# frutiemax92/YAT

Measured on AMD Instinct MI355X. Metric: images/sec (whole node) SANA-1.6B 1024px bf16 training step, higher is better.
Workload: dtype bf16; 1 GPU; train_sana.py: SANA-1.6B (D=2240, 20 blocks) 1024px, bf16, full fine-tune, cached latents/text embeds, aspect buckets [(32, 32), (16, 64), (24, 42), (44, 22)] round-robin, prompts of 20..300 tokens (text rows packed: the masked padding rows to T=512 are not computed), AdamW+clip; global_batch=8, per_gpu_batch=8, seq_len=1024, parallelism=dp1, num_layers=20, params=1604462784

## Files before the change

### include/yat_hip.h

```cpp
#ifndef YAT_HIP_H
#define YAT_HIP_H
#include <stdint.h>
#ifdef __cplusplus
extern "C" {
#endif

typedef void* yat_stream_t;

#define YAT_OK 0
#define YAT_EINVAL (-1)
#define YAT_ENOCOMM (-2)
#define YAT_ECOMM_BASE 1000

int yat_version(void);

typedef struct yat_gemm_epilogue {
    uint32_t struct_size;
    const void* bias;
    void* aux_out;
    int activation;
    const void* gate;
    const void* residual;
    int ld_aux, ld_gate, ld_residual, rows_per_batch;
    const void* glu_u;
// ... 125 lines not shown
int yat_add_pos_embed(int64_t rows, int N, int D, const void* x, const float* pos, void* out, yat_stream_t stream);
int yat_ddpm_add_noise(int B, int64_t per_sample, const void* x, const void* noise, const void* sqrt_alpha_prod,
                       const void* sqrt_one_minus_alpha_prod, void* noisy, yat_stream_t stream);
int yat_mse_bf16_chunk(int B, int64_t used, int64_t stride, const void* pred, const void* target, float gscale, float* loss,
                       void* dpred, float* workspace_256, yat_stream_t stream);

int yat_hadamard_scale(int rows, int cols, const void* a, int lda, const void* b, int ldb, float scale, void* out, int ldo,
                       yat_stream_t stream);
int yat_hadamard_bwd(int rows, int cols, const void* dd, int ldd, const void* a1, int ld1, const void* a2, int ld2, float scale,
                     void* t1, int ldt1, void* t2, int ldt2, yat_stream_t stream);

int yat_dora_delta(int rows, int cols, const void* W, int ldw, const void* lw, int ldl, const void* mag, float scaling,
                   void* delta, int ldd, float* s_buf, float* n_buf, yat_stream_t stream);
int yat_dora_bwd(int rows, int cols, const void* dd, int ldd, const void* W, int ldw, const void* lw, int ldl, float scaling,
                 const float* s_buf, const float* n_buf, void* t1, int ldt, void* dmag, yat_stream_t stream);

int yat_qknorm_concat_fwd(int B, int N, int T, int H, int dh, float eps, const void* qkv_img, int ld_img, const void* qkv_txt,
                          int ld_txt, const void* wq_img, const void* wk_img, const void* wq_txt, const void* wk_txt,
                          void* joint, int ld_joint, float* rstd, yat_stream_t stream);
uint64_t yat_qknorm_concat_bwd_workspace_bytes(int B, int N, int T, int dh);
int yat_qknorm_concat_bwd(int B, int N, int T, int H, int dh, const void* qkv_img, int ld_img, const void* qkv_txt, int ld_txt,
                          const void* wq_img, const void* wk_img, const void* wq_txt, const void* wk_txt, const float* rstd,
                          const void* d_joint, int ld_dj, void* dqkv_img, int ld_dimg, void* dqkv_txt, int ld_dtxt,
                          void* dwq_img, void* dwk_img, void* dwq_txt, void* dwk_txt, int accumulate_dw, void* workspace,
                          yat_stream_t stream);
int yat_joint_rows(int B, int N, int T, int C, void* joint, int ld_joint, void* img, int ld_img, void* txt, int ld_txt,
                   int to_joint, yat_stream_t stream);

uint64_t yat_gradnorm_workspace_bytes(int64_t n, int nseg);
int yat_gradnorm_clip(int64_t n, const void* grad, int nseg, const int64_t* seg_start, float max_norm, float* norm_out,
                      float* clip_coef, void* workspace, yat_stream_t stream);
int yat_gradnorm_pieces_partial(const void* grad, int npiece, const int64_t* piece_start, const int* chunk_base,
                                int max_piece_chunks, const unsigned char* owned, float* partial, yat_stream_t stream);
int yat_gradnorm_pieces_finish(int ntensor, const int* tensor_first_piece, const int* chunk_base, const float* partial,
                               float max_norm, float* norm_out, float* clip_coef, yat_stream_t stream);
int yat_adamw_step(int64_t n, void* param, void* grad, void* exp_avg, void* exp_avg_sq, const float* clip_coef,
                   double lr, double beta1, double beta2, double eps, double weight_decay, int step, int zero_grad,
                   void* ema_shadow, double ema_decay, int background, yat_stream_t stream);

int yat_dcae_conv3x3(int B, int H, int W, int Cin, int Cout, int upsample, int silu, const void* x, const void* w,
                     const void* bias, int shortcut_mode, const void* shortcut, int shortcut_channels, const void* residual,
                     int out_nchw, void* y, yat_stream_t stream);
int yat_dcae_msla_aggregate(int B, int H, int W, int C3, const void* qkv, const void* w_dw, const void* w_pw, void* out,
                            yat_stream_t stream);
int yat_dcae_rmsnorm_bias(int M, int D, float eps, const void* x, const void* w, const void* b, const void* residual,
                          int relu, void* y, yat_stream_t stream);
int yat_dcae_image_to_uint8(int64_t n, const void* x, void* out, yat_stream_t stream);

int yat_dcae_conv3x3_down(int B, int H, int W, int Cin, int Cout, const void* x, const void* w, const void* bias,
                          int shortcut, void* y, yat_stream_t stream);
int yat_dcae_conv3x3_mean(int B, int H, int W, int Cin, int Cout, const void* x, const void* w, const void* bias,
                          int shortcut, void* y, yat_stream_t stream);
int yat_dcae_image_from_uint8(int64_t npix, const void* x, const void* table, void* out, yat_stream_t stream);

uint64_t yat_vae_groupnorm_workspace_bytes(int B, int HW, int C, int G);
int yat_vae_groupnorm(int B, int HW, int C, int G, float eps, const void* x, const void* w, const void* b, int silu, void* y,
                      void* workspace, yat_stream_t stream);
int yat_vae_attn_fwd(int B, int N, int dh, const void* q, const void* k, const void* v, int ld, void* out, int ldo,
                     yat_stream_t stream);

#define YAT_PLAN_MAX_ARGS 30
#define YAT_PLAN_EVENT_RECORD (-1)
#define YAT_PLAN_STREAM_WAIT_EVENT (-2)
typedef union yat_plan_arg { int64_t i; double d; void* p; } yat_plan_arg;
typedef struct yat_plan_entry { int32_t op; int32_t nargs; yat_plan_arg a[YAT_PLAN_MAX_ARGS]; } yat_plan_entry;
int yat_plan_op_id(const char* name);
// ... 24 lines not shown
```

### yat_amd/csrc/optim.hip

```cpp
#include "common.hpp"
#include "../../include/yat_hip.h"
#include <math.h>

namespace {

constexpr int64_t NORM_CHUNK = 1 << 18;

__global__ __launch_bounds__(256) void gradnorm_partial_kernel(const bf16_t* g, const int64_t* seg_start, int maxchunks,
                                                               float* partial) {
    const int seg = blockIdx.y, ck = blockIdx.x;
    const int64_t s0 = seg_start[seg], s1 = seg_start[seg + 1];
    const int64_t c0 = s0 + (int64_t)ck * NORM_CHUNK;
    if (c0 >= s1) return;
    const int64_t c1 = (c0 + NORM_CHUNK < s1) ? c0 + NORM_CHUNK : s1;
    float s = 0.f;
    const int64_t nvec = (c1 - c0) >> 3;
    for (int64_t i = threadIdx.x; i < nvec; i += 256) {
        float v[8];
        unpack8(*reinterpret_cast<const u32x4*>(g + c0 + i * 8), v);
#pragma unroll
        for (int e = 0; e < 8; ++e) s += v[e] * v[e];
    }
    for (int64_t i = c0 + (nvec << 3) + threadIdx.x; i < c1; i += 256) { const float v = bf2f(g[i]); s += v * v; }
    __shared__ float red[4];
    s = wave_sum(s);
    if ((threadIdx.x & 63) == 0) red[threadIdx.x >> 6] = s;
    __syncthreads();
    if (threadIdx.x == 0) partial[(int64_t)seg * maxchunks + ck] = red[0] + red[1] + red[2] + red[3];
}

__global__ __launch_bounds__(256) void gradnorm_final_kernel(int nseg, const int64_t* seg_start, int maxchunks,
                                                             const float* partial, float max_norm, float* norm_out,
                                                             float* clip_coef) {
    float acc = 0.f;
    for (int seg = threadIdx.x; seg < nseg; seg += 256) {
        const int64_t len = seg_start[seg + 1] - seg_start[seg];
        const int nck = (int)((len + NORM_CHUNK - 1) / NORM_CHUNK);
        float s = 0.f;
        for (int c = 0; c < nck; ++c) s += partial[(int64_t)seg * maxchunks + c];
        const float nb = rbf(sqrtf(s));
        acc += nb * nb;
    }
    __shared__ float red[4];
    acc = wave_sum(acc);
    if ((threadIdx.x & 63) == 0) red[threadIdx.x >> 6] = acc;
    __syncthreads();
    if (threadIdx.x == 0) {
        const float total = rbf(sqrtf(red[0] + red[1] + red[2] + red[3]));
        float coef = rbf(max_norm / rbf(total + 1e-6f));
        coef = coef > 1.0f ? 1.0f : coef;
        norm_out[0] = total;
        clip_coef[0] = coef;
    }
}

__global__ __launch_bounds__(256) void gradnorm_pieces_partial_kernel(const bf16_t* g, const int64_t* piece_start,
                                                                      const int* chunk_base, const unsigned char* owned,
                                                                      float* partial) {
    const int pc = blockIdx.y, ck = blockIdx.x;
    const int nck = chunk_base[pc + 1] - chunk_base[pc];
    if (ck >= nck) return;
    float* dst = partial + chunk_base[pc] + ck;
    if (owned && !owned[pc]) {
        if (threadIdx.x == 0) *dst = 0.f;
        return;
    }
    const int64_t s1 = piece_start[pc + 1];
    const int64_t c0 = piece_start[pc] + (int64_t)ck * NORM_CHUNK;
    const int64_t c1 = (c0 + NORM_CHUNK < s1) ? c0 + NORM_CHUNK : s1;
    float s = 0.f;
    const int64_t nvec = (c1 - c0) >> 3;
    for (int64_t i = threadIdx.x; i < nvec; i += 256) {
        float v[8];
        unpack8(*reinterpret_cast<const u32x4*>(g + c0 + i * 8), v);
#pragma unroll
        for (int e = 0; e < 8; ++e) s += v[e] * v[e];
    }
    for (int64_t i = c0 + (nvec << 3) + threadIdx.x; i < c1; i += 256) { const float v = bf2f(g[i]); s += v * v; }
    __shared__ float red[4];
    s = wave_sum(s);
    if ((threadIdx.x & 63) == 0) red[threadIdx.x >> 6] = s;
    __syncthreads();
    if (threadIdx.x == 0) *dst = red[0] + red[1] + red[2] + red[3];
}

__global__ __launch_bounds__(256) void gradnorm_pieces_final_kernel(int ntensor, const int* tensor_first_piece,
                                                                    const int* chunk_base, const float* partial,
                                                                    float max_norm, float* norm_out, float* clip_coef) {
    float acc = 0.f;
    for (int t = threadIdx.x; t < ntensor; t += 256) {
        float s = 0.f;
        for (int pc = tensor_first_piece[t]; pc < tensor_first_piece[t + 1]; ++pc) {
            float sp = 0.f;
            for (int c = chunk_base[pc]; c < chunk_base[pc + 1]; ++c) sp += partial[c];
            s += sp;
        }
        const float nb = rbf(sqrtf(s));
        acc += nb * nb;
    }
    __shared__ float red[4];
    acc = wave_sum(acc);
    if ((threadIdx.x & 63) == 0) red[threadIdx.x >> 6] = acc;
    __syncthreads();
    if (threadIdx.x == 0) {
        const float total = rbf(sqrtf(red[0] + red[1] + red[2] + red[3]));
        float coef = rbf(max_norm / rbf(total + 1e-6f));
        coef = coef > 1.0f ? 1.0f : coef;
        norm_out[0] = total;
        clip_coef[0] = coef;
    }
}

struct AdamP {
    float wd_mul, w1, beta2, om_b2, bc2_sqrt, eps, neg_step_size, ema_omd;
    int use_wd, zero_grad;
};

__device__ __forceinline__ void adamw_elem(float& pr, float g, float& mr_, float& vr_, float coef, bool clip, const AdamP& a) {
    const float gr = clip ? rbf(g * coef) : g;
    if (a.use_wd) pr = rbf(pr * a.wd_mul);
    const float mr = rbf(mr_ + a.w1 * (gr - mr_));
    float vr = rbf(vr_ * a.beta2);
    vr = rbf(vr + a.om_b2 * gr * gr);
    float den = rbf(sqrtf(vr));
    den = rbf(den / a.bc2_sqrt);
    den = rbf(den + a.eps);
    pr = rbf(pr + a.neg_step_size * mr / den);
// ... 84 lines not shown
        if (a.zero_grad) *reinterpret_cast<u32x2*>(g + i * 4) = u32x2{0u, 0u};
    }
}

}

extern "C" {

static int norm_maxchunks(int64_t n) { return (int)((n + NORM_CHUNK - 1) / NORM_CHUNK); }

uint64_t yat_gradnorm_workspace_bytes(int64_t n, int nseg) {
    return (uint64_t)nseg * norm_maxchunks(n) * sizeof(float);
}

int yat_gradnorm_clip(int64_t n, const void* grad, int nseg, const int64_t* seg_start, float max_norm, float* norm_out,
                      float* clip_coef, void* workspace, yat_stream_t stream) {
    if (n <= 0 || nseg <= 0 || nseg > 65535 || !grad || !seg_start || !norm_out || !clip_coef || !workspace)
        return YAT_EINVAL;
    const int mc = norm_maxchunks(n);
    hipLaunchKernelGGL(gradnorm_partial_kernel, dim3(mc, nseg), dim3(256), 0, (hipStream_t)stream, (const bf16_t*)grad,
                       seg_start, mc, (float*)workspace);
    YAT_CHECK_LAUNCH();
    hipLaunchKernelGGL(gradnorm_final_kernel, dim3(1), dim3(256), 0, (hipStream_t)stream, nseg, seg_start, mc,
                       (const float*)workspace, max_norm, norm_out, clip_coef);
    YAT_CHECK_LAUNCH();
    return YAT_OK;
}

int yat_gradnorm_pieces_partial(const void* grad, int npiece, const int64_t* piece_start, const int* chunk_base,
                                int max_piece_chunks, const unsigned char* owned, float* partial, yat_stream_t stream) {
    if (!grad || npiece <= 0 || npiece > 65535 || !piece_start || !chunk_base || max_piece_chunks <= 0 || !partial)
        return YAT_EINVAL;
    hipLaunchKernelGGL(gradnorm_pieces_partial_kernel, dim3(max_piece_chunks, npiece), dim3(256), 0, (hipStream_t)stream,
                       (const bf16_t*)grad, piece_start, chunk_base, owned, partial);
    YAT_CHECK_LAUNCH();
    return YAT_OK;
}

int yat_gradnorm_pieces_finish(int ntensor, const int* tensor_first_piece, const int* chunk_base, const float* partial,
                               float max_norm, float* norm_out, float* clip_coef, yat_stream_t stream) {
    if (ntensor <= 0 || !tensor_first_piece || !chunk_base || !partial || !norm_out || !clip_coef) return YAT_EINVAL;
    hipLaunchKernelGGL(gradnorm_pieces_final_kernel, dim3(1), dim3(256), 0, (hipStream_t)stream, ntensor, tensor_first_piece,
                       chunk_base, partial, max_norm, norm_out, clip_coef);
    YAT_CHECK_LAUNCH();
    return YAT_OK;
}

int yat_adamw_step(int64_t n, void* param, void* grad, void* exp_avg, void* exp_avg_sq, const float* clip_coef, double lr,
                   double beta1, double beta2, double eps, double weight_decay, int step, int zero_grad, void* ema_shadow,
                   double ema_decay, int background, yat_stream_t stream) {
    if (n <= 0 || (n & 7) || step < 1 || !param || !grad || !exp_avg || !exp_avg_sq) return YAT_EINVAL;
    const double dlr = lr, db1 = beta1, db2 = beta2;
    AdamP a;
    a.use_wd = weight_decay != 0.0;
    a.wd_mul = (float)(1.0 - dlr * weight_decay);
    a.w1 = (float)(1.0 - db1);
    a.beta2 = (float)db2;
    a.om_b2 = (float)(1.0 - db2);
    const double bc1 = 1.0 - pow(db1, (double)step), bc2 = 1.0 - pow(db2, (double)step);
    a.bc2_sqrt = (float)sqrt(bc2);
    a.neg_step_size = (float)(-(dlr / bc1));
    a.eps = (float)eps;
    a.ema_omd = (float)(1.0 - ema_decay);
    a.zero_grad = zero_grad;
    if (background) {
        const int64_t nvec4 = n >> 2;
        int64_t nbg = (nvec4 + 255) / 256;
// ... 26 lines not shown
```

### yat_amd/flat.py

```python
from __future__ import annotations

import math
import os
from types import SimpleNamespace

import torch
import torch.nn as nn

from . import ops

BF16 = torch.bfloat16


class _Node(nn.Module):
    """Anonymous container so parameter names can carry the diffusers dotted paths."""


def schedule(chains):
    serial = os.environ.get("YAT_SERIAL", "0") != "0"
    return (not serial), (1 if serial else int(chains))


def isolate_streams():
    import torch.distributed as dist
# ... 39 lines not shown


class FlatParamModule(nn.Module):
    def _alloc_flat(self, specs, device, bucket_first=None):
        self.dev = torch.device(device)
        offs, off = [], 0
        for name, shape in specs:
            if bucket_first is not None and bucket_first(name):
                off = (off + SHARD_ALIGN - 1) // SHARD_ALIGN * SHARD_ALIGN
            offs.append(off)
            off += (math.prod(shape) + 7) // 8 * 8
        if bucket_first is not None:
            off = (off + SHARD_ALIGN - 1) // SHARD_ALIGN * SHARD_ALIGN
        self.numel_flat = off
        self.flat_param = torch.zeros(off, dtype=BF16, device=self.dev)
        self._grad_store = torch.zeros(off + GRAD_TAIL, dtype=BF16, device=self.dev)
        self.flat_grad = self._grad_store[:off]
        self.grad_tail = self._grad_store[off:]
        self.seg_start = torch.tensor(offs + [off], dtype=torch.int64)
        self._seg_numel = [math.prod(s) for _, s in specs]
        self.P, self.G = {}, {}
        for (name, shape), o in zip(specs, offs):
            n = math.prod(shape)
            param = nn.Parameter(self.flat_param[o:o + n].view(shape))
            param.grad = self.flat_grad[o:o + n].view(shape)
            self._register(name, param)
            self.P[name], self.G[name] = param.data, param.grad
        self._offset = dict(zip([n for n, _ in specs], offs))
        self.grad_ready = None
        self.loss_ready = None
        self.adapters = None
        self.param_events = None
        self.accumulate_grads = False
        self._arena, self._chains, self._side = {}, {}, None
        self._consts, self._plans = {}, {}
        self.use_plans = os.environ.get("YAT_LAUNCH_PLANS", "1") != "0"
        self.plan_dynamic = {}
        self._saved = None
        self._anchor = torch.zeros((), device=self.dev, requires_grad=True)
        self.gradient_checkpointing = False
        return offs, off

    def _register(self, dotted, param):
        mod = self
        parts = dotted.split(".")
        for part in parts[:-1]:
            if not hasattr(mod, part):
                mod.add_module(part, _Node())
            mod = getattr(mod, part)
        mod.register_parameter(parts[-1], param)

    def _block_buckets(self, specs, offs, total, num_layers, first_key="scale_shift_table"):
        names = [n for n, _ in specs]
        starts = [0]
        for i in range(num_layers):
            starts.append(offs[names.index(f"transformer_blocks.{i}.{first_key}")])
        return [(starts[i], starts[i + 1]) for i in range(len(starts) - 1)] + [(starts[-1], total)]

    @property
    def dtype(self):
        return BF16

    @property
    def device(self):
        return self.dev

# ... 62 lines not shown
                continue
            on_dev = t.device.type == self.dev.type and (self.dev.index is None or t.device.index == self.dev.index)
            if not on_dev or t.dtype != dtype or not t.is_contiguous():
                raise ValueError(f"forward_device: `{name}` must be a contiguous {dtype} tensor on {self.dev} "
                                 f"(got {t.dtype} on {t.device}, contiguous={t.is_contiguous()})")

    def _ev_record(self, stream):
        ev = torch.cuda.Event()
        ev.record(stream)
        if ops.RECORDER is not None:
            ops.RECORDER.entries.append(["ev_record", ev, stream])
        return ev

    def _ev_wait(self, stream, ev):
        stream.wait_event(ev)
        if ops.RECORDER is not None:
            ops.RECORDER.entries.append(["wait_event", stream, ev])

    def _wait_stream(self, waiter, waited):
        waiter.wait_stream(waited)
        if ops.RECORDER is not None:
            ops.RECORDER.entries.append(["wait_stream", waiter, waited])

    def _callback(self, fn, *args):
        fn(*args)
        if ops.RECORDER is not None:
            st = torch.cuda.current_stream()

            def again(st=st, fn=fn, args=args):
                with torch.cuda.stream(st):
                    fn(*args)
            ops.RECORDER.entries.append(["py", again])

    def _fused(self, first_key, rows_total, cols=None):
        o = self._offset[first_key]
        if cols is None:
            return self.flat_param[o:o + rows_total], self.flat_grad[o:o + rows_total]
        n = rows_total * cols
        return self.flat_param[o:o + n].view(rows_total, cols), self.flat_grad[o:o + n].view(rows_total, cols)

    def join_pending_update(self):
        pev, self.param_events = self.param_events, None
        if pev is not None:
            cur = torch.cuda.current_stream()
            for ev in pev:
                cur.wait_event(ev)

    def _chain_stream(self, c):
        if c not in self._chains:
            self._chains[c] = compute_stream(self.flat_param.device)
        return self._chains[c]

    def _side_stream(self):
        if self._side is None:
            self._side = compute_stream(self.flat_param.device, "side")
        return self._side
```

### yat_amd/lib.py

```python
from __future__ import annotations

import ctypes as C
import os

_HERE = os.path.dirname(os.path.abspath(__file__))
LIB_PATH = os.environ.get("YAT_HIP_LIB") or os.path.join(_HERE, "libyat_hip.so")

P, I, I64, U64, F, D = C.c_void_p, C.c_int, C.c_int64, C.c_uint64, C.c_float, C.c_double


class GemmEpilogue(C.Structure):
    _fields_ = [("struct_size", C.c_uint32), ("bias", P), ("aux_out", P), ("activation", I), ("gate", P), ("residual", P),
                ("ld_aux", I), ("ld_gate", I), ("ld_residual", I), ("rows_per_batch", I),
                ("glu_u", P), ("ld_glu_u", I), ("pre_add", P), ("ld_pre_add", I), ("dact_z", P), ("ld_dact_z", I),
                ("a_rowsum_out", P), ("a_rowsum_accumulate", I), ("a2", P), ("b2", P), ("k2", I), ("a2_group_n", I)]


    def __init__(self, *args, **kw):
        super().__init__(C.sizeof(GemmEpilogue), *args, **kw)


class PlanArg(C.Union):
    _fields_ = [("i", C.c_int64), ("d", C.c_double), ("p", C.c_void_p)]

# ... 41 lines not shown
    "yat_act_fwd": (I, [I64, I, P, P, P]),
    "yat_act_bwd": (I, [I64, I, P, P, P, P]),
    "yat_add_bf16": (I, [I64, P, P, P, P]),
    "yat_f32_to_bf16": (I, [I64, P, P, P]),
    "yat_memset_zero": (I, [P, U64, P]),
    "yat_transpose_bf16": (I, [I, I, I, P, P, P]),
    "yat_timestep_embed_fwd": (I, [I, I, P, P, P]),
    "yat_pad_mask": (I, [I, I, I, P, P, P, P, P, P, P]),
    "yat_pack_mask": (I, [I, I, I, I, P, P, P, P, P, P, P]),
    "yat_flow_mix": (I, [I, I64, P, P, P, P, P, P]),
    "yat_mse_fwd_bwd": (I, [I64, P, P, F, P, P, P, P]),
    "yat_lokr_rows": (I, [I64, I, I, I, P, P, P, P]),
    "yat_lokr_rows_fwd_flat": (I, [I64, I, I, I, P, P, P, I, P]),
    "yat_dropout": (I, [I64, F, U64, I, P, P, P]),
    "yat_lora_scatter_b": (I, [I, I, I, F, P, P, P, P]),
    "yat_rank_expand": (I, [I64, I, I, P, P, P, I, F, I, P]),
    "yat_lokr_small_wgrad_workspace_bytes": (U64, [I64, I, I]),
    "yat_lokr_small_wgrad": (I, [I64, I, I, I, P, P, I, P, I, F, I, P, P]),
    "yat_patch_rearrange": (I, [I, I, I, I, I, I, I, P, P, P]),
    "yat_add_pos_embed": (I, [I64, I, I, P, P, P, P]),
    "yat_ddpm_add_noise": (I, [I, I64, P, P, P, P, P, P]),
    "yat_mse_bf16_chunk": (I, [I, I64, I64, P, P, F, P, P, P, P]),
    "yat_hadamard_scale": (I, [I, I, P, I, P, I, F, P, I, P]),
    "yat_hadamard_bwd": (I, [I, I, P, I, P, I, P, I, F, P, I, P, I, P]),
    "yat_dora_delta": (I, [I, I, P, I, P, I, P, F, P, I, P, P, P]),
    "yat_dora_bwd": (I, [I, I, P, I, P, I, P, I, F, P, P, P, I, P, P]),
    "yat_qknorm_concat_fwd": (I, [I, I, I, I, I, F, P, I, P, I, P, P, P, P, P, I, P, P]),
    "yat_qknorm_concat_bwd_workspace_bytes": (U64, [I, I, I, I]),
    "yat_qknorm_concat_bwd": (I, [I, I, I, I, I, P, I, P, I, P, P, P, P, P, P, I, P, I, P, I, P, P, P, P, I, P, P]),
    "yat_joint_rows": (I, [I, I, I, I, P, I, P, I, P, I, I, P]),
    "yat_gradnorm_workspace_bytes": (U64, [I64, I]),
    "yat_gradnorm_clip": (I, [I64, P, I, P, F, P, P, P, P]),
    "yat_gradnorm_pieces_partial": (I, [P, I, P, P, I, P, P, P]),
    "yat_gradnorm_pieces_finish": (I, [I, P, P, P, F, P, P, P]),
    "yat_adamw_step": (I, [I64, P, P, P, P, P, D, D, D, D, D, I, I, P, D, I, P]),
    "yat_dcae_conv3x3": (I, [I, I, I, I, I, I, I, P, P, P, I, P, I, P, I, P, P]),
    "yat_dcae_msla_aggregate": (I, [I, I, I, I, P, P, P, P, P]),
    "yat_dcae_rmsnorm_bias": (I, [I, I, F, P, P, P, P, I, P, P]),
    "yat_dcae_image_to_uint8": (I, [I64, P, P, P]),
    "yat_dcae_conv3x3_down": (I, [I, I, I, I, I, P, P, P, I, P, P]),
    "yat_dcae_conv3x3_mean": (I, [I, I, I, I, I, P, P, P, I, P, P]),
    "yat_dcae_image_from_uint8": (I, [I64, P, P, P, P]),
    "yat_vae_groupnorm_workspace_bytes": (U64, [I, I, I, I]),
    "yat_vae_groupnorm": (I, [I, I, I, I, F, P, P, P, I, P, P, P]),
    "yat_vae_attn_fwd": (I, [I, I, I, P, P, P, I, P, I, P]),
    "yat_plan_op_id": (I, [C.c_char_p]),
    "yat_plan_replay": (I, [C.POINTER(PlanEntry), I, C.POINTER(I)]),
    "yat_comm_available": (I, []),
    "yat_comm_unique_id": (I, [P]),
    "yat_comm_init": (I, [I, I, P]),
    "yat_comm_world": (I, []),
    "yat_comm_rank": (I, []),
    "yat_comm_broadcast": (I, [P, U64, I, P]),
    "yat_bucket_allreduce_async": (I, [P, U64, I, P, P]),
    "yat_comm_allreduce": (I, [P, U64, I, I, P]),
    "yat_bucket_reduce_scatter_async": (I, [P, U64, I, P, P]),
    "yat_comm_allgather": (I, [P, U64, P]),
    "yat_comm_wait": (I, [I, P]),
    "yat_comm_destroy": (I, []),
    "yat_comm_last_error": (C.c_char_p, []),
}


class YatLibraryError(RuntimeError):
    pass

# ... 35 lines not shown
```

### yat_amd/ops.py

```python
from __future__ import annotations

import contextlib
import ctypes as C
import os

import torch

from . import lib as _l

BF16 = torch.bfloat16
ACT = {"none": 0, "silu": 1, "gelu_tanh": 2}

_GEMM_WS = {}
GEMM_WS_BYTES = 96 << 20


def _gemm_ws(device):
    key = (device, torch.cuda.current_stream().cuda_stream)
    ws = _GEMM_WS.get(key)
    if ws is None:
        ws = torch.empty(GEMM_WS_BYTES, dtype=torch.uint8, device=device)
        _GEMM_WS[key] = ws
    return ws

# ... 638 lines not shown
                                     _p(noisy), _stream()), "ddpm_add_noise")
    return noisy


def mse_bf16_chunk(pred, target, loss_f32, dpred, workspace_f32, gscale=1.0):
    _chk_bf16(pred, target)
    B = pred.shape[0]
    stride, used = pred.numel() // B, target.numel() // B
    if target.shape[0] != B or used > stride or pred.shape[2:] != target.shape[2:] or workspace_f32.numel() < 256 \
            or not (pred.is_contiguous() and target.is_contiguous()) or (dpred is not None and dpred.shape != pred.shape):
        raise ValueError("mse_bf16_chunk: shape mismatch")
    _l.check(_lib().yat_mse_bf16_chunk(B, used, stride, _p(pred), _p(target), float(gscale), _p(loss_f32),
                                     _p(dpred) if dpred is not None else None, _p(workspace_f32), _stream()), "mse_bf16_chunk")
    return loss_f32


def gradnorm_workspace_bytes(n, nseg):
    return int(_lib().yat_gradnorm_workspace_bytes(n, nseg))


def gradnorm_clip(grad_flat, seg_start_i64, max_norm, norm_out, clip_coef, workspace):
    nseg = seg_start_i64.numel() - 1
    rc = _lib().yat_gradnorm_clip(grad_flat.numel(), _p(grad_flat), nseg, _p(seg_start_i64), max_norm, _p(norm_out),
                                  _p(clip_coef), _p(workspace), _stream())
    _l.check(rc, "yat_gradnorm_clip")


def gradnorm_pieces_partial(grad_flat, piece_start_i64, chunk_base_i32, max_piece_chunks, owned_u8, partial_f32):
    rc = _lib().yat_gradnorm_pieces_partial(_p(grad_flat), piece_start_i64.numel() - 1, _p(piece_start_i64), _p(chunk_base_i32),
                                            int(max_piece_chunks), _p(owned_u8), _p(partial_f32), _stream())
    _l.check(rc, "yat_gradnorm_pieces_partial")


def gradnorm_pieces_finish(tensor_first_piece_i32, chunk_base_i32, partial_f32, max_norm, norm_out, clip_coef):
    rc = _lib().yat_gradnorm_pieces_finish(tensor_first_piece_i32.numel() - 1, _p(tensor_first_piece_i32), _p(chunk_base_i32),
                                           _p(partial_f32), float(max_norm), _p(norm_out), _p(clip_coef), _stream())
    _l.check(rc, "yat_gradnorm_pieces_finish")


def adamw_step(param, grad, exp_avg, exp_avg_sq, clip_coef, lr, beta1, beta2, eps, weight_decay, step, zero_grad=True,
               ema_shadow=None, ema_decay=0.0, background=0):
    rc = _lib().yat_adamw_step(param.numel(), _p(param), _p(grad), _p(exp_avg), _p(exp_avg_sq), _p(clip_coef), lr, beta1,
                               beta2, eps, weight_decay, step, int(zero_grad), _p(ema_shadow), ema_decay, int(background),
                               _stream())
    _l.check(rc, "yat_adamw_step")


def dcae_conv3x3(x, w, y, B, H, W, Cin, Cout, bias=None, upsample=False, silu=False, shortcut_mode=0, shortcut=None,
                 shortcut_channels=0, residual=None, out_nchw=False):
    _chk_bf16(x, w, y, bias, shortcut, residual)
    rc = _lib().yat_dcae_conv3x3(B, H, W, Cin, Cout, int(upsample), int(silu), _p(x), _p(w), _p(bias), int(shortcut_mode),
                                 _p(shortcut), int(shortcut_channels), _p(residual), int(out_nchw), _p(y), _stream())
    _l.check(rc, "yat_dcae_conv3x3")
    return y


def dcae_msla_aggregate(qkv, w_dw, w_pw, out, B, H, W, C3):
    _chk_bf16(qkv, w_dw, w_pw, out)
    rc = _lib().yat_dcae_msla_aggregate(B, H, W, C3, _p(qkv), _p(w_dw), _p(w_pw), _p(out), _stream())
    _l.check(rc, "yat_dcae_msla_aggregate")
    return out


def dcae_rmsnorm_bias(x2d, w, b, y, eps=1e-5, residual=None, relu=False):
    _chk_bf16(x2d, w, b, y, residual)
    M, D = x2d.shape
# ... 66 lines not shown
```

### yat_amd/optim.py

```python
from __future__ import annotations

import os

import torch

from . import ops

BF16 = torch.bfloat16


NORM_CHUNK = 1 << 18
NORM_PARTS = 8


def norm_pieces(seg_start, bucket_bounds, parts=NORM_PARTS):
    seg = [int(x) for x in seg_start]
    cuts, part_of = set(), []
    for bi, (lo, hi) in enumerate(bucket_bounds):
        L = hi - lo
        cuts.add(lo)
        if L > 0 and L % (8 * parts) == 0:
            cuts.update(lo + k * (L // parts) for k in range(1, parts))
    cuts = sorted(cuts)
    piece_start, tensor_first = [], []
    import bisect
    for t in range(len(seg) - 1):
        s0, s1 = seg[t], seg[t + 1]
        tensor_first.append(len(piece_start))
        if s1 <= s0:
            continue
        inner = cuts[bisect.bisect_right(cuts, s0):bisect.bisect_left(cuts, s1)]
        piece_start.extend([s0] + inner)
    tensor_first.append(len(piece_start))
    piece_start.append(seg[-1])
    lows = [lo for lo, _ in bucket_bounds]
    for p0 in piece_start[:-1]:
        bi = max(0, bisect.bisect_right(lows, p0) - 1)
        lo, hi = bucket_bounds[bi]
        L = hi - lo
        part_of.append((bi, (p0 - lo) // (L // parts)) if (L > 0 and L % (8 * parts) == 0) else (bi, -1))
    chunk_base, mx = [0], 1
    for a, b in zip(piece_start[:-1], piece_start[1:]):
        n = (b - a + NORM_CHUNK - 1) // NORM_CHUNK
        chunk_base.append(chunk_base[-1] + n)
        mx = max(mx, n)
    return piece_start, tensor_first, chunk_base, mx, part_of


class FlatAdamW:
    def __init__(self, model, lr, weight_decay=0.0, betas=(0.9, 0.999), eps=1e-8, max_grad_norm=1.0, use_ema=False,
                 ema_decay=0.999, overlap_update=False):
        self.model = model
        dev = model.flat_param.device
        self.param_groups = [dict(lr=lr, initial_lr=lr, weight_decay=weight_decay, betas=betas, eps=eps)]
        self.max_grad_norm = max_grad_norm
        self.exp_avg = torch.zeros_like(model.flat_param)
        self.exp_avg_sq = torch.zeros_like(model.flat_param)
        self.step_count = 0
        self.seg_start = model.seg_start.to(dev)
        ps, tf, cb, self._max_chunks, self._piece_part = norm_pieces(model.seg_start.tolist(), list(model.bucket_bounds))
        self._piece_start = torch.tensor(ps, dtype=torch.int64, device=dev)
        self._tensor_first = torch.tensor(tf, dtype=torch.int32, device=dev)
        self._chunk_base = torch.tensor(cb, dtype=torch.int32, device=dev)
        self._partial = torch.zeros(cb[-1], dtype=torch.float32, device=dev)
        self._owned, self._owned_for = None, None
        self.grad_norm = torch.zeros(1, dtype=torch.float32, device=dev)
        self.clip_coef = torch.ones(1, dtype=torch.float32, device=dev)
        self.ema_shadow = model.flat_param.clone() if use_ema else None
        self.ema_decay = ema_decay
        self.ema_steps = 0
        self.overlap_update = overlap_update and dev.type == "cuda"
        self.background_blocks = 0
        self._stream = None

    def _ema_decay_now(self):
        step = max(0, self.ema_steps - 1)
        if step <= 0:
            return 0.0
        return max(min((1 + step) / (10 + step), self.ema_decay), 0.0)

    def step(self):
        g = self.param_groups[0]
        self.step_count += 1
        m = self.model
        coef = None
        shard = self._shard()
        if self.max_grad_norm is not None:
            ops.gradnorm_pieces_partial(m.flat_grad, self._piece_start, self._chunk_base, self._max_chunks,
                                        None if shard is None else self._owned_mask(shard), self._partial)
            if shard is not None:
                shard.ddp.allreduce_bulk(self._partial, mean=False)
            ops.gradnorm_pieces_finish(self._tensor_first, self._chunk_base, self._partial, float(self.max_grad_norm),
                                       self.grad_norm, self.clip_coef)
            coef = self.clip_coef
        ema_decay = 0.0
        if self.ema_shadow is not None:
            self.ema_steps += 1
            ema_decay = self._ema_decay_now()

        bg = self.background_blocks if self.overlap_update else 0

        def update(lo, hi, step_count=None):
            ops.adamw_step(m.flat_param[lo:hi], m.flat_grad[lo:hi], self.exp_avg[lo:hi], self.exp_avg_sq[lo:hi], coef,
                           g["lr"], g["betas"][0], g["betas"][1], g["eps"], g["weight_decay"],
                           self.step_count if step_count is None else step_count,
                           zero_grad=False, ema_shadow=None if self.ema_shadow is None else self.ema_shadow[lo:hi],
                           ema_decay=ema_decay, background=bg)

        ranges = getattr(m, "update_ranges", None)
        if shard is not None:
            if ranges is not None:
                raise RuntimeError("a sharded optimizer step over an adapter set with module dropout is not built")
            self._sharded_update(shard, update)
            return
        if ranges is not None:
            m.join_pending_update()
            for lo, hi, sc in ranges():
                update(lo, hi, sc)
            return
        if not self.overlap_update:
            update(0, m.numel_flat)
            return
# ... 73 lines not shown
```

### yat_amd/sana.py

```python
from __future__ import annotations

import contextlib
import math
import os
from dataclasses import dataclass, field, asdict
from types import SimpleNamespace

import torch
import torch.nn as nn

from . import ops
from .flat import FlatParamModule, schedule
from .lokr import adapted_linear

BF16 = torch.bfloat16


@dataclass
class SanaConfig:
    in_channels: int = 32
    out_channels: int = 32
    num_attention_heads: int = 70
    attention_head_dim: int = 32
    num_layers: int = 20
# ... 129 lines not shown
            self._text_rows = self.plan_dynamic["text_rows"] = int(enc.shape[0])
        key = (latents.data_ptr(), tuple(latents.shape), enc.data_ptr(), enc_shape, timestep.data_ptr(),
               key_bias.data_ptr(), kv_len.data_ptr(), None if kv_off is None else kv_off.data_ptr(),
               None if pev is None else id(pev[0]), self._schedule_flags())
        out = self.planned("fwd", key, lambda: self.forward_impl(latents, enc, timestep, None, key_bias=key_bias,
                                                                 kv_len=kv_len, kv_work=kv_work, kv_off=kv_off))
        self.param_events = None
        self._saved.kv_work = kv_work
        if kv_off is not None and self._saved.Mt != int(enc.shape[0]):
            self._retarget_text(self._saved, enc)
        return out

    def _retarget_text(self, S, enc):
        Mt, D, f32 = int(enc.shape[0]), self.cfg.inner_dim, torch.float32
        if Mt > S.Mt_cap:
            raise RuntimeError("packed text rows exceed the capacity the forward was recorded with")

        def tb(name, cols, dtype=BF16):
            return (self._buf(name, (S.Mt_cap, cols), dtype) if cols else self._buf(name, (S.Mt_cap,), dtype))[:Mt]
        S.Mt, S.enc2d = Mt, enc.view(Mt, -1)
        S.zc1, S.c1, S.c2, S.encn = tb("cap_z1", D), tb("cap_c1", D), tb("cap_c2", D), tb("cap_n", D)
        S.enc_rstd = tb("cap_rstd", 0, f32)
        S.kv2 = [tb(f"b{i}.kv2", 2 * D) for i in range(self.cfg.num_layers)]
        for A, kv in zip(S.blocks, S.kv2):
            A.kv2 = kv

    def backward_device(self, dpred):
        S = self._saved
        work = S.kv_work
        if work is not None:
            self.plan_dynamic["n_work"] = int(work.shape[0])
        if S.kv_off is not None:
            self.plan_dynamic["text_rows"] = self._text_rows
        key = (id(S), dpred.data_ptr(), self.accumulate_grads, id(self.grad_ready), None if work is None else work.data_ptr(),
               self._schedule_flags())
        self.planned("bwd", key, lambda: self.backward_impl(dpred))

    def forward_impl(self, latents, enc, timestep, mask=None, key_bias=None, kv_len=None, kv_work=None, kv_off=None):
        cfg, P = self.cfg, self.P
        D, Hc, H1, H2, dh2 = cfg.inner_dim, cfg.ffn_hidden, cfg.num_attention_heads, cfg.num_cross_attention_heads, \
            cfg.cross_attention_head_dim
        B, Cin, h, w = latents.shape
        N, M = h * w, B * h * w
        packed = kv_off is not None
        if packed and (key_bias is None or kv_len is None or enc.dim() != 2 or enc.shape[0] % 256 or not enc.shape[0]):
            raise ValueError("packed text: enc [rows, C] (rows a multiple of 256) with key_bias [B, T], kv_len [B], kv_off [B]")
        T = key_bias.shape[1] if packed else enc.shape[1]
        Mt = enc.shape[0] if packed else B * T
        Mt_cap = max(-(-(B * T) // 256) * 256 if packed else B * T, Mt)
        Cout = cfg.out_channels
        dev = self.dev
        latents = latents.to(device=dev, dtype=BF16).contiguous()
        enc2d = enc.to(device=dev, dtype=BF16).contiguous().view(Mt, -1)
        t_f32 = timestep.to(device=dev, dtype=torch.float32).contiguous()
        if key_bias is None:
            if mask is None:
                key_bias = torch.zeros(B, T, dtype=torch.float32, device=dev)
                kv_len = torch.full((B,), T, dtype=torch.int32, device=dev)
            else:
                mdev = mask.to(dev)
                key_bias = ((1 - mdev.to(BF16)) * -10000.0).float().contiguous()
                idx = torch.arange(1, T + 1, device=dev, dtype=torch.int32)
                kv_len = (mdev.to(torch.int32) * idx).amax(dim=1).to(torch.int32).contiguous()
        S = SimpleNamespace(B=B, h=h, w=w, N=N, M=M, T=T, Mt=Mt, Mt_cap=Mt_cap, key_bias=key_bias, kv_len=kv_len,
                            kv_work=kv_work, kv_off=kv_off, enc2d=enc2d, blocks=[])
        buf = self._buf

        def tbuf(name, cols, dtype=BF16):
            return buf(name, (Mt_cap, cols), dtype)[:Mt] if cols else buf(name, (Mt_cap,), dtype)[:Mt]
# ... 148 lines not shown
                    joins.append(self._ev_record(st))
            run_chain(bounds[0], bounds[1], main)
            for ev in joins:
                self._ev_wait(main, ev)
        self._saved = S
        return pred.view(B, Cout, h, w)

    def backward_impl(self, dpred):
        S = self._saved
        if S is None:
            raise RuntimeError("backward_impl called without a saved forward")
        ops.gemm_concurrency(2 if self.side_wgrad else 1)
        cfg, P, G = self.cfg, self.P, self.G
        D, Hc, H1, H2, dh2 = cfg.inner_dim, cfg.ffn_hidden, cfg.num_attention_heads, cfg.num_cross_attention_heads, \
            cfg.cross_attention_head_dim
        B, h, w, N, M, T, Mt = S.B, S.h, S.w, S.N, S.M, S.T, S.Mt
        Cout, Cin = cfg.out_channels, cfg.in_channels
        acc = self.accumulate_grads
        buf = self._buf
        packed, Mt_cap = S.kv_off is not None, S.Mt_cap

        def tbuf(name, cols, dtype=BF16):
            return buf(name, (Mt_cap, cols), dtype)[:Mt]

        text_scope = (lambda: ops.text_rows(Mt)) if packed else contextlib.nullcontext
        f32, u8 = torch.float32, torch.uint8
        ws_col = buf("ws_col", (int(ops._lib().yat_colsum_workspace_bytes(max(M, Mt_cap), max(2 * Hc, 6 * D, 3 * D))),), u8)
        ws_ln = buf("ws_ln", (ops.ln_bwd_workspace_bytes(M, D, N),), u8)
        ws_gate = buf("ws_gate", (int(ops._lib().yat_gate_bwd_workspace_bytes(M, D, N)),), u8)
        ws_dw = buf("ws_dw", (ops.dwconv_glu_bwd_workspace_bytes(B, h, w, Hc),), u8)
        la_ws = buf("la_ws", (ops.linear_attn_workspace_bytes(B, N, H1),), u8)
        scale2 = 1.0 / math.sqrt(dh2)
        ad = self.adapters

        def dgrad(dy_, w_, out=None, residual=None):
            r_ = ops.linear_dgrad(dy_, w_, out=out, residual=residual)
            if ad is not None:
                flush_adapter_wgrads(dy_, ad.dgrad_term(dy_, w_, r_))
            return r_

        pending_ad = []

        def flush_adapter_wgrads(dy_=None, hs=None):
            keep = []
            for item in pending_ad:
                if dy_ is None or item[0].data_ptr() == dy_.data_ptr():
                    run_off_chain(lambda item=item, hs=(hs if dy_ is not None else None):
                                  ad.wgrad(*item, accumulate=acc, hs=hs))
                else:
                    keep.append(item)
            pending_ad[:] = keep

        main = torch.cuda.current_stream()
        side = self._side_stream() if self.side_wgrad else None

        def run_off_chain(fn):
            if side is None:
                fn()
                return
            self._wait_stream(side, torch.cuda.current_stream())
            with torch.cuda.stream(side):
                fn()

        def wgrad(dy, x, key, shape2d, bias_key=None):
            def run():
                if ad is not None:
# ... 126 lines not shown
                ops.linear_attn_bwd(A.qkv, B, N, H1, D, 2 * D, dattn, dqkv, la_ws, state=A.la_state)
            wqkv, gqkv = self._fused(pre + "attn1.to_q.weight", 3 * D, D)
            emit(dqkv, A.h1, gqkv)
            dh1 = dgrad(dqkv, wqkv, out=buf(f"dh1.{par}", (M, D)))
            ln1 = (A.x_in, A.mean1, A.rstd1, mod2d[:, D:2 * D], 6 * D, N, dh1)
            dx = ops.ln_modulate_bwd(*ln1, dx1, dx, dmod2d[:, 0:D], dmod2d[:, D:2 * D], 6 * D, ws_ln,
                                     parts=1 if side is not None else 3)

            def table_grads(ln1=ln1, dmod=dmod, dmod2d=dmod2d, pre=pre):
                if side is not None:
                    ops.ln_modulate_bwd(*ln1, None, None, dmod2d[:, 0:D], dmod2d[:, D:2 * D], 6 * D, ws_ln, parts=2)
                ops.modulation_bwd(dmod, G[pre + "scale_shift_table"], dtmod, D, accumulate_table=acc)
            off_chain(table_grads)

            def block_grads(deferred=deferred, dx2=dx2, dq2=dq2, dkv2=dkv2, wkv=wkv, gbkv=gbkv, pre=pre,
                            first=(i == cfg.num_layers - 1)):
                if deferred:
                    for dy_, x_, gw_, _, text_ in deferred:
                        with (text_scope() if text_ else contextlib.nullcontext()):
                            ops.linear_wgrad(dy_, x_, gw_, accumulate=acc)
                    for dy_, _, _, bias_, text_ in deferred:
                        if bias_ is not None:
                            with (text_scope() if text_ else contextlib.nullcontext()):
                                ops.colsum(dy_, bias_, ws_col, accumulate=acc)
                with text_scope():
                    dgrad(dkv2, wkv, out=denc, residual=None if first else denc)

            if ad is not None:
                flush_adapter_wgrads()
            if side is None:
                block_grads()
                if self.grad_ready is not None:
                    self._callback(self.grad_ready, i + 1)
            else:
                self._wait_stream(side, main)
                with torch.cuda.stream(side):
                    block_grads()
                    if self.grad_ready is not None:
                        self._callback(self.grad_ready, i + 1)
                    set_done[par] = self._ev_record(side)
        if side is not None:
            self._wait_stream(main, side)
            side = None
        wgrad(dx, S.x_tok, "patch_embed.proj.weight", (D, Cin), "patch_embed.proj.bias")
        dc2 = tbuf("dc2", D)
        ws_rms = buf("ws_rms", (int(ops._lib().yat_rmsnorm_bwd_workspace_bytes(Mt_cap, D)),), u8)
        with text_scope():
            ops.rmsnorm_bwd(S.c2, P["caption_norm.weight"], S.enc_rstd, denc, dc2, G["caption_norm.weight"], ws_rms,
                            accumulate_dw=acc)
            wgrad(dc2, S.c1, "caption_projection.linear_2.weight", (D, D), "caption_projection.linear_2.bias")
            dc1 = dgrad(dc2, P["caption_projection.linear_2.weight"], out=denc)
            dzc1 = ops.act_bwd(S.zc1, dc1, "gelu_tanh", dc2)
            wgrad(dzc1, S.enc2d, "caption_projection.linear_1.weight", (D, cfg.caption_channels),
                  "caption_projection.linear_1.bias")
        dtmod_b = ops.f32_to_bf16(dtmod, buf("dtmod_b", (B, 6 * D)))
        wgrad(dtmod_b, S.se, "time_embed.linear.weight", (6 * D, D), "time_embed.linear.bias")
        dse = ops.linear_dgrad(dtmod_b, P["time_embed.linear.weight"], out=buf("te_d1", (B, D)))
        demb_a = ops.act_bwd(S.embedded, dse, "silu", buf("te_d2", (B, D)))
        demb_b = ops.f32_to_bf16(demb, buf("te_d3", (B, D)))
        d_emb = ops.add_bf16(demb_a, demb_b, buf("te_d1", (B, D)))
        wgrad(d_emb, S.e1, "time_embed.emb.timestep_embedder.linear_2.weight", (D, D), "time_embed.emb.timestep_embedder.linear_2.bias")
        de1 = dgrad(d_emb, P["time_embed.emb.timestep_embedder.linear_2.weight"], out=buf("te_d2", (B, D)))
        dz1 = ops.act_bwd(S.z1, de1, "silu", buf("te_d3", (B, D)))
        wgrad(dz1, S.tproj, "time_embed.emb.timestep_embedder.linear_1.weight", (D, 256), "time_embed.emb.timestep_embedder.linear_1.bias")
        if self.grad_ready is not None:
            self._callback(self.grad_ready, 0)
        if ad is not None:
            ad.project()

    def save_pretrained(self, path):
        import json
        import os
        from safetensors.torch import save_file
        os.makedirs(path, exist_ok=True)
        self.join_pending_update()
        sd = {k: v.detach().cpu().contiguous() for k, v in self.state_dict().items()}
        save_file(sd, os.path.join(path, "diffusion_pytorch_model.safetensors"))
        cfgd = asdict(self.cfg)
        cfgd.update({"_class_name": "SanaTransformer2DModel", "cross_attention_dim": self.cfg.cross_attention_dim,
                     "attention_bias": False, "dropout": 0.0, "norm_elementwise_affine": False,
                     "interpolation_scale": None})
        with open(os.path.join(path, "config.json"), "w") as f:
            json.dump(cfgd, f, indent=2)

    @classmethod
    def from_pretrained(cls, path, device="cuda", **_):
        import json
        import os
        from safetensors.torch import load_file
        with open(os.path.join(path, "config.json")) as f:
            raw = json.load(f)
        known = {k: raw[k] for k in SanaConfig.__dataclass_fields__ if k in raw}
        model = cls(SanaConfig(**known), device=device)
        model.load_state_dict(load_file(os.path.join(path, "diffusion_pytorch_model.safetensors")))
        return model
```

Before: 106.3 images/s.

## Compute grad-norm partials per bucket during backward instead of after

```diff
diff --git a/include/yat_hip.h b/include/yat_hip.h
--- a/include/yat_hip.h
+++ b/include/yat_hip.h
@@ -181,6 +181,9 @@
                       float* clip_coef, void* workspace, yat_stream_t stream);
 int yat_gradnorm_pieces_partial(const void* grad, int npiece, const int64_t* piece_start, const int* chunk_base,
                                 int max_piece_chunks, const unsigned char* owned, float* partial, yat_stream_t stream);
+int yat_gradnorm_pieces_partial_range(const void* grad, int piece_lo, int piece_hi, const int64_t* piece_start,
+                                      const int* chunk_base, int range_max_chunks, const unsigned char* owned, float* partial,
+                                      yat_stream_t stream);
 int yat_gradnorm_pieces_finish(int ntensor, const int* tensor_first_piece, const int* chunk_base, const float* partial,
                                float max_norm, float* norm_out, float* clip_coef, yat_stream_t stream);
 int yat_adamw_step(int64_t n, void* param, void* grad, void* exp_avg, void* exp_avg_sq, const float* clip_coef,
diff --git a/yat_amd/csrc/optim.hip b/yat_amd/csrc/optim.hip
--- a/yat_amd/csrc/optim.hip
+++ b/yat_amd/csrc/optim.hip
@@ -56,8 +56,8 @@
 
 __global__ __launch_bounds__(256) void gradnorm_pieces_partial_kernel(const bf16_t* g, const int64_t* piece_start,
                                                                       const int* chunk_base, const unsigned char* owned,
-                                                                      float* partial) {
-    const int pc = blockIdx.y, ck = blockIdx.x;
+                                                                      float* partial, int pc0) {
+    const int pc = pc0 + blockIdx.y, ck = blockIdx.x;
     const int nck = chunk_base[pc + 1] - chunk_base[pc];
     if (ck >= nck) return;
     float* dst = partial + chunk_base[pc] + ck;
@@ -84,15 +84,39 @@
     if (threadIdx.x == 0) *dst = red[0] + red[1] + red[2] + red[3];
 }
 
+constexpr int FINAL_LDS_CHUNKS = 10240;
+constexpr int FINAL_LDS_PIECES = 2560;
+
 __global__ __launch_bounds__(256) void gradnorm_pieces_final_kernel(int ntensor, const int* tensor_first_piece,
                                                                     const int* chunk_base, const float* partial,
                                                                     float max_norm, float* norm_out, float* clip_coef) {
+    __shared__ float lds_partial[FINAL_LDS_CHUNKS];
+    __shared__ int lds_base[FINAL_LDS_PIECES + 1];
+    __shared__ float lds_piece[FINAL_LDS_PIECES];
+    const int npiece = tensor_first_piece[ntensor];
+    const int nchunk = chunk_base[npiece];
+    const bool staged = npiece <= FINAL_LDS_PIECES && nchunk <= FINAL_LDS_CHUNKS;
+    if (staged) {
+        for (int c = threadIdx.x; c < nchunk; c += 256) lds_partial[c] = partial[c];
+        for (int p = threadIdx.x; p <= npiece; p += 256) lds_base[p] = chunk_base[p];
+        __syncthreads();
+        for (int pc = threadIdx.x; pc < npiece; pc += 256) {
+            float sp = 0.f;
+            for (int c = lds_base[pc]; c < lds_base[pc + 1]; ++c) sp += lds_partial[c];
+            lds_piece[pc] = sp;
+        }
+        __syncthreads();
+    }
     float acc = 0.f;
     for (int t = threadIdx.x; t < ntensor; t += 256) {
         float s = 0.f;
         for (int pc = tensor_first_piece[t]; pc < tensor_first_piece[t + 1]; ++pc) {
             float sp = 0.f;
-            for (int c = chunk_base[pc]; c < chunk_base[pc + 1]; ++c) sp += partial[c];
+            if (staged) {
+                sp = lds_piece[pc];
+            } else {
+                for (int c = chunk_base[pc]; c < chunk_base[pc + 1]; ++c) sp += partial[c];
+            }
             s += sp;
         }
         const float nb = rbf(sqrtf(s));
@@ -243,7 +267,19 @@
     if (!grad || npiece <= 0 || npiece > 65535 || !piece_start || !chunk_base || max_piece_chunks <= 0 || !partial)
         return YAT_EINVAL;
     hipLaunchKernelGGL(gradnorm_pieces_partial_kernel, dim3(max_piece_chunks, npiece), dim3(256), 0, (hipStream_t)stream,
-                       (const bf16_t*)grad, piece_start, chunk_base, owned, partial);
+                       (const bf16_t*)grad, piece_start, chunk_base, owned, partial, 0);
+    YAT_CHECK_LAUNCH();
+    return YAT_OK;
+}
+
+int yat_gradnorm_pieces_partial_range(const void* grad, int piece_lo, int piece_hi, const int64_t* piece_start,
+                                      const int* chunk_base, int range_max_chunks, const unsigned char* owned, float* partial,
+                                      yat_stream_t stream) {
+    if (!grad || piece_lo < 0 || piece_hi <= piece_lo || piece_hi - piece_lo > 65535 || !piece_start || !chunk_base ||
+        range_max_chunks <= 0 || !partial)
+        return YAT_EINVAL;
+    hipLaunchKernelGGL(gradnorm_pieces_partial_kernel, dim3(range_max_chunks, piece_hi - piece_lo), dim3(256), 0,
+                       (hipStream_t)stream, (const bf16_t*)grad, piece_start, chunk_base, owned, partial, piece_lo);
     YAT_CHECK_LAUNCH();
     return YAT_OK;
 }
diff --git a/yat_amd/flat.py b/yat_amd/flat.py
--- a/yat_amd/flat.py
+++ b/yat_amd/flat.py
@@ -95,6 +95,9 @@
         self.adapters = None
         self.param_events = None
         self.accumulate_grads = False
+        self.bucket_norm = None
+        self.norm_fresh = None
+        self.norm_late = os.environ.get("YAT_NORM_BUCKETED", "1") == "late"
         self._arena, self._chains, self._side = {}, {}, None
         self._consts, self._plans = {}, {}
         self.use_plans = os.environ.get("YAT_LAUNCH_PLANS", "1") != "0"
@@ -223,6 +226,14 @@
                     fn(*args)
             ops.RECORDER.entries.append(["py", again])
 
+    def _bucket_norm_hook(self):
+        if self.accumulate_grads or self.grad_ready is not None or self.adapters is not None:
+            return None
+        return self.bucket_norm
+
+    def _mark_norm(self, hook):
+        self.norm_fresh = None if hook is None else (hook, self.flat_grad._version)
+
     def _fused(self, first_key, rows_total, cols=None):
         o = self._offset[first_key]
         if cols is None:
diff --git a/yat_amd/lib.py b/yat_amd/lib.py
--- a/yat_amd/lib.py
+++ b/yat_amd/lib.py
@@ -97,6 +97,7 @@
     "yat_gradnorm_workspace_bytes": (U64, [I64, I]),
     "yat_gradnorm_clip": (I, [I64, P, I, P, F, P, P, P, P]),
     "yat_gradnorm_pieces_partial": (I, [P, I, P, P, I, P, P, P]),
+    "yat_gradnorm_pieces_partial_range": (I, [P, I, I, P, P, I, P, P, P]),
     "yat_gradnorm_pieces_finish": (I, [I, P, P, P, F, P, P, P]),
     "yat_adamw_step": (I, [I64, P, P, P, P, P, D, D, D, D, D, I, I, P, D, I, P]),
     "yat_dcae_conv3x3": (I, [I, I, I, I, I, I, I, P, P, P, I, P, I, P, I, P, P]),
diff --git a/yat_amd/ops.py b/yat_amd/ops.py
--- a/yat_amd/ops.py
+++ b/yat_amd/ops.py
@@ -694,6 +694,16 @@
     _l.check(rc, "yat_gradnorm_pieces_partial")
 
 
+def gradnorm_pieces_partial_range(grad_flat, piece_lo, piece_hi, piece_start_i64, chunk_base_i32, range_max_chunks, owned_u8,
+                                  partial_f32):
+    if not 0 <= piece_lo < piece_hi <= piece_start_i64.numel() - 1:
+        raise ValueError(f"gradnorm_pieces_partial_range: pieces [{piece_lo}, {piece_hi}) of {piece_start_i64.numel() - 1}")
+    rc = _lib().yat_gradnorm_pieces_partial_range(_p(grad_flat), int(piece_lo), int(piece_hi), _p(piece_start_i64),
+                                                  _p(chunk_base_i32), int(range_max_chunks), _p(owned_u8), _p(partial_f32),
+                                                  _stream())
+    _l.check(rc, "yat_gradnorm_pieces_partial_range")
+
+
 def gradnorm_pieces_finish(tensor_first_piece_i32, chunk_base_i32, partial_f32, max_norm, norm_out, clip_coef):
     rc = _lib().yat_gradnorm_pieces_finish(tensor_first_piece_i32.numel() - 1, _p(tensor_first_piece_i32), _p(chunk_base_i32),
                                            _p(partial_f32), float(max_norm), _p(norm_out), _p(clip_coef), _stream())
diff --git a/yat_amd/optim.py b/yat_amd/optim.py
--- a/yat_amd/optim.py
+++ b/yat_amd/optim.py
@@ -47,6 +47,20 @@
     return piece_start, tensor_first, chunk_base, mx, part_of
 
 
+def bucket_piece_ranges(piece_start, chunk_base, bucket_bounds):
+    import bisect
+    starts = piece_start[:-1]
+    out = []
+    for lo, hi in bucket_bounds:
+        p0, p1 = bisect.bisect_left(starts, lo), bisect.bisect_left(starts, hi)
+        if p0 < p1 and (piece_start[p0] != lo or piece_start[p1] > hi):
+            raise ValueError("norm pieces straddle a bucket boundary")
+        out.append((p0, p1, max([chunk_base[p + 1] - chunk_base[p] for p in range(p0, p1)], default=0)))
+    if [r[0] for r in out[1:]] != [r[1] for r in out[:-1]] or out[0][0] != 0 or out[-1][1] != len(starts):
+        raise ValueError("the buckets' piece ranges do not tile the pieces")
+    return out
+
+
 class FlatAdamW:
     def __init__(self, model, lr, weight_decay=0.0, betas=(0.9, 0.999), eps=1e-8, max_grad_norm=1.0, use_ema=False,
                  ema_decay=0.999, overlap_update=False):
@@ -64,6 +78,12 @@
         self._chunk_base = torch.tensor(cb, dtype=torch.int32, device=dev)
         self._partial = torch.zeros(cb[-1], dtype=torch.float32, device=dev)
         self._owned, self._owned_for = None, None
+        self._bucket_ranges = bucket_piece_ranges(ps, cb, list(model.bucket_bounds))
+        self._norm_hook = self.bucket_norm
+        if os.environ.get("YAT_NORM_BUCKETED", "1") != "0" and dev.type == "cuda" and max_grad_norm is not None \
+                and hasattr(model, "norm_fresh"):
+            model.bucket_norm, model.norm_fresh = self._norm_hook, None
+            model._plans.clear()
         self.grad_norm = torch.zeros(1, dtype=torch.float32, device=dev)
         self.clip_coef = torch.ones(1, dtype=torch.float32, device=dev)
         self.ema_shadow = model.flat_param.clone() if use_ema else None
@@ -79,6 +99,20 @@
             return 0.0
         return max(min((1 + step) / (10 + step), self.ema_decay), 0.0)
 
+    def bucket_norm(self, bucket):
+        p0, p1, mx = self._bucket_ranges[bucket]
+        if p0 < p1:
+            ops.gradnorm_pieces_partial_range(self.model.flat_grad, p0, p1, self._piece_start, self._chunk_base, mx, None,
+                                              self._partial)
+
+    def _partials_fresh(self, shard):
+        m = self.model
+        mark = getattr(m, "norm_fresh", None)
+        if mark is None:
+            return False
+        m.norm_fresh = None
+        return shard is None and mark[0] is self._norm_hook and mark[1] == m.flat_grad._version
+
     def step(self):
         g = self.param_groups[0]
         self.step_count += 1
@@ -86,8 +120,9 @@
         coef = None
         shard = self._shard()
         if self.max_grad_norm is not None:
-            ops.gradnorm_pieces_partial(m.flat_grad, self._piece_start, self._chunk_base, self._max_chunks,
-                                        None if shard is None else self._owned_mask(shard), self._partial)
+            if not self._partials_fresh(shard):
+                ops.gradnorm_pieces_partial(m.flat_grad, self._piece_start, self._chunk_base, self._max_chunks,
+                                            None if shard is None else self._owned_mask(shard), self._partial)
             if shard is not None:
                 shard.ddp.allreduce_bulk(self._partial, mean=False)
             ops.gradnorm_pieces_finish(self._tensor_first, self._chunk_base, self._partial, float(self.max_grad_norm),
diff --git a/yat_amd/sana.py b/yat_amd/sana.py
--- a/yat_amd/sana.py
+++ b/yat_amd/sana.py
@@ -185,9 +185,11 @@
             self.plan_dynamic["n_work"] = int(work.shape[0])
         if S.kv_off is not None:
             self.plan_dynamic["text_rows"] = self._text_rows
+        hook = self._bucket_norm_hook()
         key = (id(S), dpred.data_ptr(), self.accumulate_grads, id(self.grad_ready), None if work is None else work.data_ptr(),
-               self._schedule_flags())
+               self._schedule_flags(), id(hook), self.norm_late)
         self.planned("bwd", key, lambda: self.backward_impl(dpred))
+        self._mark_norm(hook)
 
     def forward_impl(self, latents, enc, timestep, mask=None, key_bias=None, kv_len=None, kv_work=None, kv_off=None):
         cfg, P = self.cfg, self.P
@@ -402,6 +404,20 @@
         la_ws = buf("la_ws", (ops.linear_attn_workspace_bytes(B, N, H1),), u8)
         scale2 = 1.0 / math.sqrt(dh2)
         ad = self.adapters
+        norm_hook = self._bucket_norm_hook()
+        self.norm_fresh = None
+        norm_due = []
+
+        def bucket_norm(bucket):
+            if norm_hook is None:
+                return
+            if self.norm_late and bucket:
+                norm_due.append(bucket)
+                bucket = norm_due.pop(0) if len(norm_due) > 1 else None
+            elif norm_due:
+                norm_hook(norm_due.pop())
+            if bucket is not None:
+                norm_hook(bucket)
 
         def dgrad(dy_, w_, out=None, residual=None):
             r_ = ops.linear_dgrad(dy_, w_, out=out, residual=residual)
@@ -594,12 +610,14 @@
                 block_grads()
                 if self.grad_ready is not None:
                     self._callback(self.grad_ready, i + 1)
+                bucket_norm(i + 1)
             else:
                 self._wait_stream(side, main)
                 with torch.cuda.stream(side):
                     block_grads()
                     if self.grad_ready is not None:
                         self._callback(self.grad_ready, i + 1)
+                    bucket_norm(i + 1)
                     set_done[par] = self._ev_record(side)
         if side is not None:
             self._wait_stream(main, side)
@@ -627,6 +645,8 @@
         wgrad(dz1, S.tproj, "time_embed.emb.timestep_embedder.linear_1.weight", (D, 256), "time_embed.emb.timestep_embedder.linear_1.bias")
         if self.grad_ready is not None:
             self._callback(self.grad_ready, 0)
+        bucket_norm(0)
+        self._mark_norm(norm_hook)
         if ad is not None:
             ad.project()
 
```

Measured after the change: 106.4 images/s (median of 4 runs). About the same (+0.1%).
